# HITSZ-NRSL/De6D

Measured on AMD Instinct MI355X. Metric: scenes/sec (16384-pt KITTI) at 1/2/4/8 MI355X; 3D mAP parity vs ref, higher is better.
Workload: dtype f32

## Files before the change

### de6d_amd/csrc/fps_multi.h

```cpp
#pragma once
#include "fps_common.h"

namespace {

constexpr int kCandMax = 4;
constexpr int kWaves = 16, kSlots = 16;
constexpr int kMaxPicks = 32;
constexpr int kCoopMaxPicks = 64;
static_assert(kWaves * kCandMax == 64, "one sequencer lane per candidate");

template <int LO, int HI, int N>
__device__ __forceinline__ void sq_select(int ws, const float (&px)[N], const float (&py)[N], const float (&pz)[N],
                                          float &x, float &y, float &z) {
  if constexpr (HI - LO == 1) {
    x = px[LO]; y = py[LO]; z = pz[LO];
    asm volatile("" : "+v"(x), "+v"(y), "+v"(z));
  } else {
    constexpr int MID = (LO + HI) / 2;
    if (ws < MID) sq_select<LO, MID>(ws, px, py, pz, x, y, z);
    else sq_select<MID, HI>(ws, px, py, pz, x, y, z);
  }
}

template <int LO, int HI, int N>
__device__ __forceinline__ void sq_select5(int ws, const float (&px)[N], const float (&py)[N], const float (&pz)[N],
                                           const float (&pt)[N], const float (&pw)[N], float &x, float &y, float &z, float &t, float &w) {
  if constexpr (HI - LO == 1) {
    x = px[LO]; y = py[LO]; z = pz[LO]; t = pt[LO]; w = pw[LO];
    asm volatile("" : "+v"(x), "+v"(y), "+v"(z), "+v"(t), "+v"(w));
  } else {
    constexpr int MID = (LO + HI) / 2;
    if (ws < MID) sq_select5<LO, MID>(ws, px, py, pz, pt, pw, x, y, z, t, w);
    else sq_select5<MID, HI>(ws, px, py, pz, pt, pw, x, y, z, t, w);
  }
}

__device__ __forceinline__ void sq_quad_max2(float a, float b, float &ra, float &rb) {
  asm volatile(
      "s_nop 1\n\t"
      "v_max_f32_dpp %0, %2, %2 quad_perm:[1,0,3,2] row_mask:0xf bank_mask:0xf\n\t"
      "v_max_f32_dpp %1, %3, %3 quad_perm:[1,0,3,2] row_mask:0xf bank_mask:0xf\n\t"
      "s_nop 0\n\t"
      "v_max_f32_dpp %0, %0, %0 quad_perm:[2,3,0,1] row_mask:0xf bank_mask:0xf\n\t"
      "v_max_f32_dpp %1, %1, %1 quad_perm:[2,3,0,1] row_mask:0xf bank_mask:0xf\n\t"
      "s_nop 1\n\t"
      : "=&v"(ra), "=&v"(rb)
      : "v"(a), "v"(b));
}

__device__ __forceinline__ float sq_quad_max(float a) {
  float r;
  asm volatile(
      "s_nop 1\n\t"
      "v_max_f32_dpp %0, %1, %1 quad_perm:[1,0,3,2] row_mask:0xf bank_mask:0xf\n\t"
      "s_nop 1\n\t"
      "v_max_f32_dpp %0, %0, %0 quad_perm:[2,3,0,1] row_mask:0xf bank_mask:0xf\n\t"
      "s_nop 1\n\t"
      : "=&v"(r)
      : "v"(a));
  return r;
}

__device__ __forceinline__ float sq_pair_max(float a) {
  float r;
  asm volatile(
      "s_nop 1\n\t"
      "v_max_f32_dpp %0, %1, %1 quad_perm:[1,0,3,2] row_mask:0xf bank_mask:0xf\n\t"
      "s_nop 1\n\t"
      : "=&v"(r)
      : "v"(a));
  return r;
}
template <int K, int N>
__device__ __forceinline__ void sq_group_max_n(const float (&a)[N], float (&r)[N]) {
  static_assert(N == 1 || N == 2 || N == 4, "values per call");
  if constexpr (N == 4) {
    if constexpr (K == 2) {
      asm volatile("s_nop 1\n\t"
                   "v_max_f32_dpp %0, %4, %4 quad_perm:[1,0,3,2] row_mask:0xf bank_mask:0xf\n\t"
                   "v_max_f32_dpp %1, %5, %5 quad_perm:[1,0,3,2] row_mask:0xf bank_mask:0xf\n\t"
                   "v_max_f32_dpp %2, %6, %6 quad_perm:[1,0,3,2] row_mask:0xf bank_mask:0xf\n\t"
                   "v_max_f32_dpp %3, %7, %7 quad_perm:[1,0,3,2] row_mask:0xf bank_mask:0xf\n\t"
                   "s_nop 1\n\t"
                   : "=&v"(r[0]), "=&v"(r[1]), "=&v"(r[2]), "=&v"(r[3])
                   : "v"(a[0]), "v"(a[1]), "v"(a[2]), "v"(a[3]));
    } else {
      asm volatile("s_nop 1\n\t"
                   "v_max_f32_dpp %0, %4, %4 quad_perm:[1,0,3,2] row_mask:0xf bank_mask:0xf\n\t"
                   "v_max_f32_dpp %1, %5, %5 quad_perm:[1,0,3,2] row_mask:0xf bank_mask:0xf\n\t"
                   "v_max_f32_dpp %2, %6, %6 quad_perm:[1,0,3,2] row_mask:0xf bank_mask:0xf\n\t"
                   "v_max_f32_dpp %3, %7, %7 quad_perm:[1,0,3,2] row_mask:0xf bank_mask:0xf\n\t"
                   "v_max_f32_dpp %0, %0, %0 quad_perm:[2,3,0,1] row_mask:0xf bank_mask:0xf\n\t"
                   "v_max_f32_dpp %1, %1, %1 quad_perm:[2,3,0,1] row_mask:0xf bank_mask:0xf\n\t"
                   "v_max_f32_dpp %2, %2, %2 quad_perm:[2,3,0,1] row_mask:0xf bank_mask:0xf\n\t"
                   "v_max_f32_dpp %3, %3, %3 quad_perm:[2,3,0,1] row_mask:0xf bank_mask:0xf\n\t"
                   "s_nop 1\n\t"
                   : "=&v"(r[0]), "=&v"(r[1]), "=&v"(r[2]), "=&v"(r[3])
                   : "v"(a[0]), "v"(a[1]), "v"(a[2]), "v"(a[3]));
    }
  } else if constexpr (N == 2) {
    if constexpr (K == 2) {
      asm volatile("s_nop 1\n\t"
                   "v_max_f32_dpp %0, %2, %2 quad_perm:[1,0,3,2] row_mask:0xf bank_mask:0xf\n\t"
                   "v_max_f32_dpp %1, %3, %3 quad_perm:[1,0,3,2] row_mask:0xf bank_mask:0xf\n\t"
                   "s_nop 1\n\t"
                   : "=&v"(r[0]), "=&v"(r[1]) : "v"(a[0]), "v"(a[1]));
    } else {
      sq_quad_max2(a[0], a[1], r[0], r[1]);
    }
  } else {
    if constexpr (K == 2) r[0] = sq_pair_max(a[0]);
    else r[0] = sq_quad_max(a[0]);
  }
}

template <int K>
__device__ __forceinline__ float sq_group_max(float a) {
  if constexpr (K == 2) return sq_pair_max(a);
  else return sq_quad_max(a);
}

template <int K>
__device__ __forceinline__ unsigned sq_group_max_u32(unsigned a) {
  unsigned r;
  if constexpr (K == 2)
    asm volatile("s_nop 1\n\t"
                 "v_max_u32_dpp %0, %1, %1 quad_perm:[1,0,3,2] row_mask:0xf bank_mask:0xf\n\t"
                 "s_nop 1\n\t"
                 : "=&v"(r) : "v"(a));
  else
    asm volatile("s_nop 1\n\t"
                 "v_max_u32_dpp %0, %1, %1 quad_perm:[1,0,3,2] row_mask:0xf bank_mask:0xf\n\t"
                 "s_nop 1\n\t"
                 "v_max_u32_dpp %0, %0, %0 quad_perm:[2,3,0,1] row_mask:0xf bank_mask:0xf\n\t"
                 "s_nop 1\n\t"
                 : "=&v"(r) : "v"(a));
  return r;
}

__device__ __forceinline__ unsigned sq_wave_max_u32(unsigned v) {
  unsigned t;
  asm volatile(
      "s_nop 1\n\t"
      "v_max_u32_dpp %0, %1, %1 quad_perm:[1,0,3,2] row_mask:0xf bank_mask:0xf\n\t"
      "s_nop 1\n\t"
      "v_max_u32_dpp %0, %0, %0 quad_perm:[2,3,0,1] row_mask:0xf bank_mask:0xf\n\t"
      "s_nop 1\n\t"
      "v_max_u32_dpp %0, %0, %0 row_half_mirror row_mask:0xf bank_mask:0xf\n\t"
      "s_nop 1\n\t"
      "v_max_u32_dpp %0, %0, %0 row_mirror row_mask:0xf bank_mask:0xf\n\t"
      "s_nop 1\n\t"
      "v_max_u32_dpp %0, %0, %0 row_bcast:15 row_mask:0xa bank_mask:0xf\n\t"
      "s_nop 1\n\t"
      "v_max_u32_dpp %0, %0, %0 row_bcast:31 row_mask:0xc bank_mask:0xf\n\t"
      "s_nop 1\n\t"
      : "=&v"(t)
      : "v"(v));
  return (unsigned)__builtin_amdgcn_readlane((int)t, 63);
}

__device__ __forceinline__ void sq_wave_max2(float a, float b, float &ra, float &rb) {
  float ta, tb;
  asm volatile(
      "s_nop 1\n\t"
      "v_max_f32_dpp %0, %2, %2 quad_perm:[1,0,3,2] row_mask:0xf bank_mask:0xf\n\t"
      "v_max_f32_dpp %1, %3, %3 quad_perm:[1,0,3,2] row_mask:0xf bank_mask:0xf\n\t"
      "s_nop 0\n\t"
      "v_max_f32_dpp %0, %0, %0 quad_perm:[2,3,0,1] row_mask:0xf bank_mask:0xf\n\t"
      "v_max_f32_dpp %1, %1, %1 quad_perm:[2,3,0,1] row_mask:0xf bank_mask:0xf\n\t"
      "s_nop 0\n\t"
      "v_max_f32_dpp %0, %0, %0 row_half_mirror row_mask:0xf bank_mask:0xf\n\t"
      "v_max_f32_dpp %1, %1, %1 row_half_mirror row_mask:0xf bank_mask:0xf\n\t"
      "s_nop 0\n\t"
      "v_max_f32_dpp %0, %0, %0 row_mirror row_mask:0xf bank_mask:0xf\n\t"
      "v_max_f32_dpp %1, %1, %1 row_mirror row_mask:0xf bank_mask:0xf\n\t"
      "s_nop 0\n\t"
      "v_max_f32_dpp %0, %0, %0 row_bcast:15 row_mask:0xa bank_mask:0xf\n\t"
      "v_max_f32_dpp %1, %1, %1 row_bcast:15 row_mask:0xa bank_mask:0xf\n\t"
      "s_nop 0\n\t"
      "v_max_f32_dpp %0, %0, %0 row_bcast:31 row_mask:0xc bank_mask:0xf\n\t"
      "v_max_f32_dpp %1, %1, %1 row_bcast:31 row_mask:0xc bank_mask:0xf\n\t"
      "s_nop 1\n\t"
      : "=&v"(ta), "=&v"(tb)
      : "v"(a), "v"(b));
  ra = d6_readlane_f(ta, 63);
  rb = d6_readlane_f(tb, 63);
}

struct SqRecords {
  float v[64], x[64], y[64], z[64];
  int k[64];
  int nc[kWaves];
};

struct SqRecordsW {
  float t[64], w[64];
};

template <int SG>
__device__ __forceinline__ void sq_hide_lane_duplicates(const float (&px)[SG], const float (&py)[SG], const float (&pz)[SG],
                                                        float (&pt)[SG]) {
#pragma unroll
  for (int j = 1; j < SG; ++j) {
    bool dup = false;
#pragma unroll
    for (int i = 0; i < j; ++i) dup |= px[i] == px[j] && py[i] == py[j] && pz[i] == pz[j];
    pt[j] = dup ? 0.f : pt[j];
  }
}

template <int SG>
__device__ __forceinline__ void sq_hide_lane_duplicates_w(const float (&px)[SG], const float (&py)[SG], const float (&pz)[SG],
                                                          const float (&pw)[SG], float (&pt)[SG]) {
#pragma unroll
  for (int j = 1; j < SG; ++j) {
    bool dup = false;
#pragma unroll
    for (int i = 0; i < j; ++i) dup |= px[i] == px[j] && py[i] == py[j] && pz[i] == pz[j] && pw[i] == pw[j];
    pt[j] = dup ? 0.f : pt[j];
  }
}

template <int SG>
__device__ __forceinline__ void sq_apply(float cx, float cy, float cz, const float (&px)[SG], const float (&py)[SG],
                                         const float (&pz)[SG], float (&pt)[SG]) {
  const fps_f32x2 c2x = {cx, cx}, c2y = {cy, cy}, c2z = {cz, cz};
#pragma unroll
  for (int q = 0; q < SG / 2; ++q) {
    const int s0 = 2 * q;
    const fps_f32x2 dx = fps_f32x2{px[s0], px[s0 + 1]} - c2x;
    const fps_f32x2 dy = fps_f32x2{py[s0], py[s0 + 1]} - c2y;
    const fps_f32x2 dz = fps_f32x2{pz[s0], pz[s0 + 1]} - c2z;
    fps_f32x2 d = dy * dy;
    d = __builtin_elementwise_fma(dx, dx, d);
    d = __builtin_elementwise_fma(dz, dz, d);
    pt[s0] = d6_vmin(d[0], pt[s0]);
    pt[s0 + 1] = d6_vmin(d[1], pt[s0 + 1]);
  }
}

template <int SG, int kCand>
__device__ __forceinline__ float sq_rescan(float cx, float cy, float cz, int log2s, const float (&px)[SG], const float (&py)[SG],
                                           const float (&pz)[SG], float (&pt)[SG], const unsigned short *korig_w, SqRecords &rec,
                                           int wave, int depth = kCand) {
  const int lane = threadIdx.x & 63;
  float best = -1.0f, sec = -1.0f;
  int bs = 0;
  const fps_f32x2 c2x = {cx, cx}, c2y = {cy, cy}, c2z = {cz, cz};
  auto visit = [&](int j, float d) {
    const float t = d6_vmin(d, pt[j]);
    pt[j] = t;
    sec = __builtin_amdgcn_fmed3f(best, sec, t);
    const bool up = t > best;
    bs = up ? j : bs;
    best = d6_vmax(best, t);
  };
#pragma unroll
  for (int q = 0; q < SG / 2; ++q) {
    const int s0 = 2 * q;
    const fps_f32x2 dx = fps_f32x2{px[s0], px[s0 + 1]} - c2x;
    const fps_f32x2 dy = fps_f32x2{py[s0], py[s0 + 1]} - c2y;
    const fps_f32x2 dz = fps_f32x2{pz[s0], pz[s0 + 1]} - c2z;
    fps_f32x2 d = dy * dy;
    d = __builtin_elementwise_fma(dx, dx, d);
    d = __builtin_elementwise_fma(dz, dz, d);
    visit(s0, d[0]);
    visit(s0 + 1, d[1]);
  }
  static_assert(SG % 2 == 0, "slot pairs");
  auto second_slot = [&]() -> int {
    float target = sec;
    int skip = bs;
    asm volatile("" : "+v"(target), "+v"(skip));
    int ss = 0;
#pragma unroll
    for (int j = SG - 1; j >= 0; --j) ss = (pt[j] == target && j != skip) ? j : ss;
    return ss;
  };

  int taken = 0;
  float head = best;
  float cmax = 0.f;
  int nc = 0;
#pragma nounroll
  for (int i = 0; i < depth; ++i) {
    const float wm = d6_wave_max(head);
    if (i == 0) cmax = wm;
    const u64 tie = __ballot(head == wm);
    int wl = __builtin_ctzll(tie);
    int ss = 0;
    bool have_ss = false;
    if (__popcll(tie) != 1) {
      if (__ballot(taken != 0 && head == wm) != 0ull) { ss = second_slot(); have_ss = true; }
      const int hs = taken ? ss : bs;
      wl = fps_min_key_lane(tie, fps_tie_key((int)korig_w[lane * SG + hs], log2s));
    }
    const int wtk = d6_readlane_i(taken, wl);
    int ws;
    if (wtk == 0) {
      ws = d6_readlane_i(bs, wl);
    } else {
      if (!have_ss) ss = second_slot();
      ws = d6_readlane_i(ss, wl);
    }
    if (lane == wl) {
      float x, y, z;
      sq_select<0, SG>(ws, px, py, pz, x, y, z);
      const int o = wave * kCandMax + i;
      rec.v[o] = wm;
      rec.k[o] = (int)korig_w[lane * SG + ws];
      rec.x[o] = x; rec.y[o] = y; rec.z[o] = z;
      taken = 1;
      head = sec;
    }
    nc = i + 1;
    if (wtk != 0) break;
  }
  if (lane == 0) rec.nc[wave] = nc;
  return cmax;
}

template <int SG, int kCand>
__device__ __forceinline__ float sq_rescan_w(float cx, float cy, float cz, int log2s, const float (&px)[SG], const float (&py)[SG],
                                             const float (&pz)[SG], const float (&pw)[SG], float (&pt)[SG],
                                             const unsigned short *korig_w, SqRecords &rec, SqRecordsW &recw, int wave,
                                             int depth = kCand) {
  const int lane = threadIdx.x & 63;
  float best = -1.0f, sec = -1.0f, tm = 0.f;
  int bs = 0;
  const fps_f32x2 c2x = {cx, cx}, c2y = {cy, cy}, c2z = {cz, cz};
  auto visit = [&](int j, float d) {
    const float t = d6_vmin(d, pt[j]);
    pt[j] = t;
    tm = d6_vmax(tm, t);
    const float sc = t * pw[j];
    sec = __builtin_amdgcn_fmed3f(best, sec, sc);
    const bool up = sc > best;
    bs = up ? j : bs;
    best = d6_vmax(best, sc);
  };
#pragma unroll
  for (int q = 0; q < SG / 2; ++q) {
    const int s0 = 2 * q;
    const fps_f32x2 dx = fps_f32x2{px[s0], px[s0 + 1]} - c2x;
    const fps_f32x2 dy = fps_f32x2{py[s0], py[s0 + 1]} - c2y;
    const fps_f32x2 dz = fps_f32x2{pz[s0], pz[s0 + 1]} - c2z;
    fps_f32x2 d = dy * dy;
    d = __builtin_elementwise_fma(dx, dx, d);
    d = __builtin_elementwise_fma(dz, dz, d);
    visit(s0, d[0]);
    visit(s0 + 1, d[1]);
  }
  auto second_slot = [&]() -> int {
    float target = sec;
    int skip = bs;
    asm volatile("" : "+v"(target), "+v"(skip));
    int ss = 0;
#pragma unroll
    for (int j = SG - 1; j >= 0; --j) ss = (pt[j] * pw[j] == target && j != skip) ? j : ss;
    return ss;
  };
  int taken = 0;
  float head = best;
  int nc = 0;
#pragma nounroll
  for (int i = 0; i < depth; ++i) {
    const float wm = d6_wave_max(head);
    const u64 tie = __ballot(head == wm);
    int wl = __builtin_ctzll(tie);
    int ss = 0;
    bool have_ss = false;
    if (__popcll(tie) != 1) {
      if (__ballot(taken != 0 && head == wm) != 0ull) { ss = second_slot(); have_ss = true; }
      const int hs = taken ? ss : bs;
      wl = fps_min_key_lane(tie, fps_tie_key((int)korig_w[lane * SG + hs], log2s));
    }
    const int wtk = d6_readlane_i(taken, wl);
    int ws;
    if (wtk == 0) {
      ws = d6_readlane_i(bs, wl);
    } else {
      if (!have_ss) ss = second_slot();
      ws = d6_readlane_i(ss, wl);
    }
    if (lane == wl) {
      float x, y, z, t, w;
      sq_select5<0, SG>(ws, px, py, pz, pt, pw, x, y, z, t, w);
      const int o = wave * kCandMax + i;
      rec.v[o] = wm;
      rec.k[o] = (int)korig_w[lane * SG + ws];
      rec.x[o] = x; rec.y[o] = y; rec.z[o] = z;
      recw.t[o] = t; recw.w[o] = w;
      taken = 1;
      head = sec;
    }
    nc = i + 1;
    if (wtk != 0) break;
  }
  if (lane == 0) rec.nc[wave] = nc;
  return d6_wave_max(tm);
}

}
```

### de6d_amd/csrc/fps_seq.hip

```cpp
#include <stdio.h>
#include "fps_common.h"
#include "fps_multi.h"

namespace {

#ifdef DET6D_EXPERIMENTS
__device__ unsigned long long d6_fps_seq_stats[16];
#define SQ_STAT(i, v) do { const unsigned long long sv_ = (unsigned long long)(v); if (blockIdx.x == 0 && (threadIdx.x & 63) == 0) atomicAdd(&sq_stats_lds[i], sv_); } while (0)
#else
#define SQ_STAT(i, v) do { } while (0)
#endif

template <int kCand, int SG = kSlots>
__global__ __launch_bounds__(1024) void fps_seq_kernel(int n, int m, int log2s, long long xyz_bstride, long long idx_bstride,
                                                       int idx_add, const float *__restrict__ xyz,
                                                       const int *__restrict__ perm, int *__restrict__ idxs, int max_picks, int depth_add) {
  __shared__ unsigned short korig[64 * kWaves * SG];
  __shared__ SqRecords rec;
  __shared__ float pick_x[kMaxPicks], pick_y[kMaxPicks], pick_z[kMaxPicks];
  __shared__ int pick_n;
#ifdef DET6D_EXPERIMENTS
  __shared__ unsigned long long sq_stats_lds[16];
  if (threadIdx.x < 16) sq_stats_lds[threadIdx.x] = 0ull;
  const long long t_begin = clock64();
#endif
  const int h = threadIdx.x, lane = h & 63;
  const int wave = __builtin_amdgcn_readfirstlane(h >> 6);
  xyz += (size_t)blockIdx.x * xyz_bstride;
  perm += (size_t)blockIdx.x * n;
  idxs += (size_t)blockIdx.x * idx_bstride;
  unsigned short *korig_w = korig + (size_t)wave * 64 * SG;

  float px[SG], py[SG], pz[SG], pt[SG];
  float lox, loy, loz, hix, hiy, hiz;
  {
    float ax = 3.0e38f, ay = 3.0e38f, az = 3.0e38f, bx = -3.0e38f, by = -3.0e38f, bz = -3.0e38f;
#pragma unroll
    for (int j = 0; j < SG; ++j) {
      const int pos = (wave * 64 + lane) * SG + j;
      const int k = perm[pos];
      korig[pos] = (unsigned short)k;
      px[j] = xyz[(size_t)k * 3 + 0];
      py[j] = xyz[(size_t)k * 3 + 1];
      pz[j] = xyz[(size_t)k * 3 + 2];
      asm volatile("" : "+v"(px[j]), "+v"(py[j]), "+v"(pz[j]));
      pt[j] = 1e10f;
      ax = d6_vmin(ax, px[j]); bx = d6_vmax(bx, px[j]);
      ay = d6_vmin(ay, py[j]); by = d6_vmax(by, py[j]);
      az = d6_vmin(az, pz[j]); bz = d6_vmax(bz, pz[j]);
    }
    lox = d6_wave_min(ax); hix = d6_wave_max(bx);
    loy = d6_wave_min(ay); hiy = d6_wave_max(by);
    loz = d6_wave_min(az); hiz = d6_wave_max(bz);
  }
  sq_hide_lane_duplicates<SG>(px, py, pz, pt);
  float cmax = __builtin_inff();
  if (h == 0) { pick_x[0] = xyz[0]; pick_y[0] = xyz[1]; pick_z[0] = xyz[2]; pick_n = 1; idxs[0] = idx_add; }
  __syncthreads();

  int r = 1;
  while (true) {
#ifdef DET6D_EXPERIMENTS
    const long long ta0 = clock64();
#endif
    {
      const int np = pick_n;
      const float sx = pick_x[lane & (kMaxPicks - 1)], sy = pick_y[lane & (kMaxPicks - 1)], sz = pick_z[lane & (kMaxPicks - 1)];
      const float gx = fmaxf(0.f, fmaxf(lox - sx, sx - hix));
      const float gy = fmaxf(0.f, fmaxf(loy - sy, sy - hiy));
      const float gz = fmaxf(0.f, fmaxf(loz - sz, sz - hiz));
      const float lb = d6_sqdist(gx, gy, gz);
      u64 need = __ballot(lane < np && (r == 1 || !(lb >= cmax)));
      if (need != 0ull) {
        while (need & (need - 1ull)) {
          const int i = __builtin_ctzll(need);
          need &= need - 1ull;
          sq_apply<SG>(d6_readlane_f(sx, i), d6_readlane_f(sy, i), d6_readlane_f(sz, i), px, py, pz, pt);
          SQ_STAT(3, 1);
        }
        const int i = __builtin_ctzll(need);
        SQ_STAT(2, 1);
        cmax = sq_rescan<SG, kCand>(d6_readlane_f(sx, i), d6_readlane_f(sy, i), d6_readlane_f(sz, i), log2s, px, py, pz, pt, korig_w, rec, wave,
                                    np <= depth_add ? min(kCand, 2) : kCand);
      }
    }
    if (r >= m) break;
#ifdef DET6D_EXPERIMENTS
    const long long ta1 = clock64();
    if (wave == 0) SQ_STAT(6, ta1 - ta0);
    if (wave == 5) SQ_STAT(7, ta1 - ta0);
#endif
    __syncthreads();
#ifdef DET6D_EXPERIMENTS
    const long long tb0 = clock64();
    if (wave == 0) SQ_STAT(8, tb0 - ta1);
#endif
    if (wave == 0) {
      SQ_STAT(0, 1);
      constexpr int LOG2K = kCand == 2 ? 1 : 2;
      const bool live = lane < kWaves * kCand;
      const int region = live ? lane >> LOG2K : 0;
      const int nc = rec.nc[region];
      const int slot = lane & (kCand - 1);
      const int o = region * kCandMax + slot;
      float cv = live && slot < nc ? rec.v[o] : -1.0f;
      const float qx = rec.x[o], qy = rec.y[o], qz = rec.z[o];
      const int kidx = rec.k[o];
      const bool is_last = live && slot == nc - 1;
      const float bound_v = sq_group_max<kCand>(is_last ? cv : -2.0f);
      const unsigned ub = ((__builtin_bit_cast(unsigned, bound_v) << 1) | 1u) + 2u;
      const bool alive = live && slot < nc;
      const unsigned ntk = ~fps_tie_key(kidx, log2s);
      const unsigned ntk_last = sq_group_max_u32<kCand>(is_last ? ntk : 0u);
      const unsigned thr = !alive ? 0xFFFFFFFFu : ntk >= ntk_last ? ub - 1u : ub;
      const unsigned alt = is_last ? ub : 0u;
      int j = 0;
      const int jmax = min(max_picks, m - r);
      int mwl = 0;
      {
        bool go;
        do {
          const unsigned ekey = (__builtin_bit_cast(unsigned, cv) << 1) + 2u;
          const unsigned key = ekey >= thr ? ekey : alt;
          const unsigned best = sq_wave_max_u32(key);
          const u64 tie = __ballot(key == best);
          int wl = __builtin_ctzll(tie);
          if (__popcll(tie) != 1) wl = fps_min_key_lane(tie, ~ntk);
          const float sx = d6_readlane_f(qx, wl), sy = d6_readlane_f(qy, wl), sz = d6_readlane_f(qz, wl);
          mwl = lane == j ? wl : mwl;
          cv = d6_vmin(cv, d6_sqdist(qx - sx, qy - sy, qz - sz));
          go = (best & 1u) == 0u;
          j += go ? 1 : 0;
#ifdef DET6D_EXPERIMENTS
          if (!go) SQ_STAT(4, 1);
#endif
        } while (go && j < jmax);
      }
      {
        const float mx = __shfl(qx, mwl), my = __shfl(qy, mwl), mz = __shfl(qz, mwl);
        const int mk = __shfl(kidx, mwl);
        if (lane < j) {
          pick_x[lane] = mx; pick_y[lane] = my; pick_z[lane] = mz;
          idxs[r + lane] = mk + idx_add;
        }
      }
      if (lane == 0) pick_n = j;
      SQ_STAT(1, j);
#ifdef DET6D_EXPERIMENTS
      SQ_STAT(9, clock64() - tb0);
#endif
    }
    __syncthreads();
    r += pick_n;
  }
#ifdef DET6D_EXPERIMENTS
  if (wave == 0) {
    SQ_STAT(5, clock64() - t_begin);
    __builtin_amdgcn_s_waitcnt(0);
    if (blockIdx.x == 0 && lane < 16) d6_fps_seq_stats[lane] = sq_stats_lds[lane];
  }
#endif
}

template <int kCand, int SG>
__global__ __launch_bounds__(1024) void fps_seq_w_kernel(int n, int m, int log2s, long long xyz_bstride, long long idx_bstride,
                                                         int idx_add, const float *__restrict__ xyz, const int *__restrict__ perm,
                                                         int *__restrict__ idxs, int max_picks, int depth_add,
                                                         const float *__restrict__ weights, long long w_bstride, float gamma,
                                                         int w_is_score, int *__restrict__ flags) {
  __shared__ unsigned short korig[64 * kWaves * SG];
  __shared__ SqRecords rec;
  __shared__ SqRecordsW recw;
  __shared__ float pick_x[kMaxPicks], pick_y[kMaxPicks], pick_z[kMaxPicks];
  __shared__ int pick_n;
  __shared__ float w0_val[kWaves], w0_x[kWaves], w0_y[kWaves], w0_z[kWaves];
  __shared__ unsigned w0_key[kWaves];
  __shared__ int small_any;
  const int h = threadIdx.x, lane = h & 63;
  const int wave = __builtin_amdgcn_readfirstlane(h >> 6);
  xyz += (size_t)blockIdx.x * xyz_bstride;
  perm += (size_t)blockIdx.x * n;
  idxs += (size_t)blockIdx.x * idx_bstride;
  weights += (size_t)blockIdx.x * w_bstride;
  flags += (size_t)blockIdx.x * n;
  unsigned short *korig_w = korig + (size_t)wave * 64 * SG;
  if (h == 0) small_any = 0;

  float px[SG], py[SG], pz[SG], pt[SG], pw[SG];
  float lox, loy, loz, hix, hiy, hiz;
  bool small = false;
  {
    float ax = 3.0e38f, ay = 3.0e38f, az = 3.0e38f, bx = -3.0e38f, by = -3.0e38f, bz = -3.0e38f;
#pragma unroll
    for (int j = 0; j < SG; ++j) {
      const int pos = (wave * 64 + lane) * SG + j;
      const int k = perm[pos];
      korig[pos] = (unsigned short)k;
      px[j] = xyz[(size_t)k * 3 + 0];
      py[j] = xyz[(size_t)k * 3 + 1];
      pz[j] = xyz[(size_t)k * 3 + 2];
      float w = weights[k];
      if (w_is_score) w = d6_sigmoid_powf(w, gamma);
      pw[j] = w;
      small = small || !((double)w >= 1e-12);
      asm volatile("" : "+v"(px[j]), "+v"(py[j]), "+v"(pz[j]), "+v"(pw[j]));
      pt[j] = 1e10f;
      ax = d6_vmin(ax, px[j]); bx = d6_vmax(bx, px[j]);
      ay = d6_vmin(ay, py[j]); by = d6_vmax(by, py[j]);
      az = d6_vmin(az, pz[j]); bz = d6_vmax(bz, pz[j]);
    }
    lox = d6_wave_min(ax); hix = d6_wave_max(bx);
    loy = d6_wave_min(ay); hiy = d6_wave_max(by);
    loz = d6_wave_min(az); hiz = d6_wave_max(bz);
  }
  __syncthreads();
  if (__ballot(small) != 0ull && lane == 0) small_any = 1;
  {
    float bw = pw[0];
    int bs0 = 0;
#pragma unroll
    for (int j = 1; j < SG; ++j) {
      const bool up = pw[j] > bw;
      bs0 = up ? j : bs0;
      bw = up ? pw[j] : bw;
    }
    const float wm = d6_wave_max(small ? 0.f : bw);
    const u64 tie = __ballot(bw == wm);
    int wl = tie ? __builtin_ctzll(tie) : 0;
    const unsigned mykey = fps_tie_key((int)korig_w[lane * SG + bs0], log2s);
    if (__popcll(tie) > 1) wl = fps_min_key_lane(tie, mykey);
    if (lane == wl) {
      float x, y, z;
      sq_select<0, SG>(bs0, px, py, pz, x, y, z);
      w0_val[wave] = bw; w0_key[wave] = mykey; w0_x[wave] = x; w0_y[wave] = y; w0_z[wave] = z;
    }
  }
  __syncthreads();
  if (h == 0) flags[0] = small_any;
  if (small_any) return;
  if (wave == 0) {
    const bool mine = lane < kWaves;
    const float v = mine ? w0_val[lane & (kWaves - 1)] : -1.0f;
    const unsigned key = mine ? w0_key[lane & (kWaves - 1)] : 0xFFFFFFFFu;
    const float vm = d6_wave_max(v);
    const u64 tie = __ballot(mine && v == vm);
    int wl = __builtin_ctzll(tie);
    if (__popcll(tie) > 1) wl = fps_min_key_lane(tie, key);
    if (lane == wl) {
      pick_x[0] = w0_x[lane]; pick_y[0] = w0_y[lane]; pick_z[0] = w0_z[lane];
      pick_n = 1;
      idxs[0] = fps_tie_key_point(key, log2s) + idx_add;
    }
  }
  sq_hide_lane_duplicates_w<SG>(px, py, pz, pw, pt);
  float cmax = __builtin_inff();
  __syncthreads();

  int r = 1;
  while (true) {
    {
      const int np = pick_n;
      const float sx = pick_x[lane & (kMaxPicks - 1)], sy = pick_y[lane & (kMaxPicks - 1)], sz = pick_z[lane & (kMaxPicks - 1)];
      const float gx = fmaxf(0.f, fmaxf(lox - sx, sx - hix));
      const float gy = fmaxf(0.f, fmaxf(loy - sy, sy - hiy));
      const float gz = fmaxf(0.f, fmaxf(loz - sz, sz - hiz));
      const float lb = d6_sqdist(gx, gy, gz);
      u64 need = __ballot(lane < np && (r == 1 || !(lb >= cmax)));
      if (need != 0ull) {
        while (need & (need - 1ull)) {
          const int i = __builtin_ctzll(need);
          need &= need - 1ull;
          sq_apply<SG>(d6_readlane_f(sx, i), d6_readlane_f(sy, i), d6_readlane_f(sz, i), px, py, pz, pt);
        }
        const int i = __builtin_ctzll(need);
        cmax = sq_rescan_w<SG, kCand>(d6_readlane_f(sx, i), d6_readlane_f(sy, i), d6_readlane_f(sz, i), log2s, px, py, pz, pw, pt, korig_w,
                                      rec, recw, wave, np <= depth_add ? min(kCand, 2) : kCand);
      }
    }
    if (r >= m) break;
    __syncthreads();
    if (wave == 0) {
      constexpr int LOG2K = kCand == 2 ? 1 : 2;
      const bool live = lane < kWaves * kCand;
      const int region = live ? lane >> LOG2K : 0;
      const int nc = rec.nc[region];
      const int slot = lane & (kCand - 1);
      const int o = region * kCandMax + slot;
      const bool alive = live && slot < nc;
      float cv = alive ? recw.t[o] : -1.0f;
      const float cw = alive ? recw.w[o] : 1.0f;
      const float sv = alive ? rec.v[o] : -1.0f;
      const float qx = rec.x[o], qy = rec.y[o], qz = rec.z[o];
      const int kidx = rec.k[o];
      const bool is_last = live && slot == nc - 1;
      const float bound_v = sq_group_max<kCand>(is_last ? sv : -2.0f);
      const unsigned ub = ((__builtin_bit_cast(unsigned, bound_v) << 1) | 1u) + 2u;
      const unsigned ntk = ~fps_tie_key(kidx, log2s);
      const unsigned ntk_last = sq_group_max_u32<kCand>(is_last ? ntk : 0u);
      const unsigned thr = !alive ? 0xFFFFFFFFu : ntk >= ntk_last ? ub - 1u : ub;
      const unsigned alt = is_last ? ub : 0u;
      int j = 0;
      const int jmax = min(max_picks, m - r);
      int mwl = 0;
      {
        bool go;
        do {
          const unsigned ekey = (__builtin_bit_cast(unsigned, cv * cw) << 1) + 2u;
          const unsigned key = ekey >= thr ? ekey : alt;
          const unsigned best = sq_wave_max_u32(key);
          const u64 tie = __ballot(key == best);
          int wl = __builtin_ctzll(tie);
          if (__popcll(tie) != 1) wl = fps_min_key_lane(tie, ~ntk);
          const float sx = d6_readlane_f(qx, wl), sy = d6_readlane_f(qy, wl), sz = d6_readlane_f(qz, wl);
          mwl = lane == j ? wl : mwl;
          cv = d6_vmin(cv, d6_sqdist(qx - sx, qy - sy, qz - sz));
          go = (best & 1u) == 0u;
          j += go ? 1 : 0;
        } while (go && j < jmax);
      }
      {
        const float mx = __shfl(qx, mwl), my = __shfl(qy, mwl), mz = __shfl(qz, mwl);
        const int mk = __shfl(kidx, mwl);
        if (lane < j) {
          pick_x[lane] = mx; pick_y[lane] = my; pick_z[lane] = mz;
          idxs[r + lane] = mk + idx_add;
        }
      }
      if (lane == 0) pick_n = j;
    }
    __syncthreads();
    r += pick_n;
  }
}

}

#ifdef DET6D_EXPERIMENTS
extern "C" __attribute__((visibility("default"))) int det6d_dbg_fps_seq_stats(unsigned long long *out_host) {
  return hipMemcpyFromSymbol(out_host, HIP_SYMBOL(d6_fps_seq_stats), sizeof(unsigned long long) * 16) == hipSuccess ? 0 : -1;
}

namespace {
__device__ unsigned d6_poison_sink;
__global__ __launch_bounds__(1024) void poison_lds_kernel(unsigned pattern, unsigned words) {
  extern __shared__ unsigned lds[];
  for (unsigned i = threadIdx.x; i < words; i += 1024) lds[i] = pattern;
  __syncthreads();
  if (lds[(threadIdx.x * 97u) % words] != pattern) d6_poison_sink = 1u;
}
}
void det6d_dbg_poison_lds_hook(hipStream_t stream) {
  static const char *env = getenv("DET6D_DBG_POISON_LDS");
  if (!env) return;
  static const unsigned pattern = (unsigned)strtoul(env, nullptr, 0);
  const unsigned bytes = 160u * 1024u;
  DET6D_MAX_DYNAMIC_LDS(poison_lds_kernel, bytes);
  hipLaunchKernelGGL(poison_lds_kernel, dim3(1024), dim3(1024), bytes, stream, pattern, bytes / 4u);
  const hipError_t rc = hipGetLastError();
  if (rc != hipSuccess) fprintf(stderr, "det6d_dbg_poison_lds_hook: %s\n", hipGetErrorString(rc));
}
namespace {
__global__ __launch_bounds__(1024) void probe_lds_kernel(unsigned *out) {
  __shared__ unsigned probe[8192];
  unsigned v = probe[threadIdx.x * 8];
  asm volatile("" : "+v"(v));
  out[blockIdx.x * 1024 + threadIdx.x] = v;
}
}
extern "C" __attribute__((visibility("default"))) int det6d_dbg_probe_lds(unsigned *out, int blocks, void *stream) {
  det6d_dbg_poison_lds_hook((hipStream_t)stream);
  hipLaunchKernelGGL(probe_lds_kernel, dim3(blocks), dim3(1024), 0, (hipStream_t)stream, out);
  return det6d_check_launch("det6d_dbg_probe_lds");
}
#endif

#ifdef DET6D_EXPERIMENTS
namespace {
template <int R>
__global__ __launch_bounds__(1024) void occupy_kernel(int usec, float *sink) {
  extern __shared__ float occ_lds[];
  float r[R];
#pragma unroll
  for (int i = 0; i < R; ++i) r[i] = (float)(threadIdx.x + i);
  const unsigned long long t0 = wall_clock64();
  while (wall_clock64() - t0 < (unsigned long long)usec * 100ull) {
    __builtin_amdgcn_s_sleep(100);
#pragma unroll
    for (int i = 0; i < R; ++i) asm volatile("" : "+v"(r[i]));
  }
  float s = 0.f;
#pragma unroll
  for (int i = 0; i < R; ++i) s += r[i];
  if (s == -1.f) { occ_lds[threadIdx.x] = s; sink[0] = occ_lds[0]; }
}
}
extern "C" __attribute__((visibility("default"))) int det6d_dbg_occupy(int blocks, int regs, int lds, int usec, float *sink, void *stream) {
  hipStream_t s = (hipStream_t)stream;
#define D6_OCC(R)                                                         \
  do {                                                                    \
    DET6D_MAX_DYNAMIC_LDS(occupy_kernel<R>, 160 * 1024);                  \
    hipLaunchKernelGGL(occupy_kernel<R>, dim3(blocks), dim3(1024), lds, s, usec, sink); \
  } while (0)
  if (regs >= 96) D6_OCC(96); else if (regs >= 80) D6_OCC(80); else if (regs >= 56) D6_OCC(56); else if (regs >= 40) D6_OCC(40); else D6_OCC(16);
#undef D6_OCC
  return det6d_check_launch("det6d_dbg_occupy");
}
#endif

int det6d_fps_seq_launch(int b, int n, int m, int log2s, long long xyz_bstride, long long idx_bstride, int idx_add,
                         const float *xyz, const int *perm, int *idx, hipStream_t stream) {
  if (n != 16384 && n != 4096) return DET6D_EINVAL;
  static const int max_picks_env = det6d_env_int("DET6D_FPS_SEQ_PICKS", kMaxPicks);
  static const int cands = det6d_env_int("DET6D_FPS_SEQ_CANDS", 4);
  static const int depth_add = det6d_env_int("DET6D_FPS_SEQ_DEPTH_ADD", 1);
  const int max_picks = max_picks_env < 1 ? 1 : max_picks_env > kMaxPicks ? kMaxPicks : max_picks_env;
#ifdef DET6D_EXPERIMENTS
  det6d_dbg_poison_lds_hook(stream);
#endif
  if (n == 4096)
    hipLaunchKernelGGL((fps_seq_kernel<4, 4>), dim3(b), dim3(1024), 0, stream, n, m, log2s, xyz_bstride, idx_bstride, idx_add, xyz, perm, idx, max_picks, depth_add);
  else if (cands == 2)
    hipLaunchKernelGGL((fps_seq_kernel<2>), dim3(b), dim3(1024), 0, stream, n, m, log2s, xyz_bstride, idx_bstride, idx_add, xyz, perm, idx, max_picks, depth_add);
  else
    hipLaunchKernelGGL((fps_seq_kernel<4>), dim3(b), dim3(1024), 0, stream, n, m, log2s, xyz_bstride, idx_bstride, idx_add, xyz, perm, idx, max_picks, depth_add);
  return det6d_check_launch("det6d_fps (multi-pick)");
}

int det6d_fps_seq_w_launch(int b, int n, int m, int log2s, long long xyz_bstride, long long idx_bstride, int idx_add,
                           const float *xyz, const int *perm, int *idx, const float *weights, long long w_bstride, float gamma,
                           int w_is_score, int *flags, hipStream_t stream) {
  if (n != 16384 && n != 4096) return DET6D_EINVAL;
  static const int max_picks_env = det6d_env_int("DET6D_FPS_SEQ_PICKS", kMaxPicks);
  static const int depth_add = det6d_env_int("DET6D_FPS_SEQ_DEPTH_ADD", 1);
  const int max_picks = max_picks_env < 1 ? 1 : max_picks_env > kMaxPicks ? kMaxPicks : max_picks_env;
#ifdef DET6D_EXPERIMENTS
  det6d_dbg_poison_lds_hook(stream);
#endif
  if (n == 4096)
    hipLaunchKernelGGL((fps_seq_w_kernel<4, 4>), dim3(b), dim3(1024), 0, stream, n, m, log2s, xyz_bstride, idx_bstride, idx_add, xyz, perm,
                       idx, max_picks, depth_add, weights, w_bstride, gamma, w_is_score, flags);
  else
    hipLaunchKernelGGL((fps_seq_w_kernel<4, 16>), dim3(b), dim3(1024), 0, stream, n, m, log2s, xyz_bstride, idx_bstride, idx_add, xyz, perm,
                       idx, max_picks, depth_add, weights, w_bstride, gamma, w_is_score, flags);
  return det6d_check_launch("det6d_fps (multi-pick, score-weighted)");
}
```

Baseline: 12780.

## Move FPS per-slot min-distances to LDS with double-buffered register staging

```diff
diff --git a/de6d_amd/csrc/fps_multi.h b/de6d_amd/csrc/fps_multi.h
--- a/de6d_amd/csrc/fps_multi.h
+++ b/de6d_amd/csrc/fps_multi.h
@@ -197,6 +197,51 @@
   float t[64], w[64];
 };
 
+constexpr int kLdsDistStride = 1024;
+constexpr int kLdsDistChunk = 4;
+struct SqLdsDist {
+  float *p;
+  float st[2 * kLdsDistChunk];
+};
+__device__ __forceinline__ constexpr int sq_stage(int j) { return ((j / kLdsDistChunk) & 1) * kLdsDistChunk + j % kLdsDistChunk; }
+
+template <int N>
+__device__ __forceinline__ float sq_dist_get(const float (&t)[N], int j) { return t[j]; }
+template <int N>
+__device__ __forceinline__ void sq_dist_set(float (&t)[N], int j, float v) { t[j] = v; }
+__device__ __forceinline__ float sq_dist_get(const SqLdsDist &t, int j) { return t.p[j * kLdsDistStride]; }
+__device__ __forceinline__ void sq_dist_set(SqLdsDist &t, int j, float v) { t.p[j * kLdsDistStride] = v; }
+
+template <int N>
+__device__ __forceinline__ void sq_sweep_open(float (&)[N]) {}
+template <int N>
+__device__ __forceinline__ float sq_sweep_get(const float (&t)[N], int j) { return t[j]; }
+template <int N>
+__device__ __forceinline__ void sq_sweep_set(float (&t)[N], int j, float v) { t[j] = v; }
+__device__ __forceinline__ void sq_sweep_open(SqLdsDist &t) {
+#pragma unroll
+  for (int j = 0; j < 2 * kLdsDistChunk; ++j) t.st[sq_stage(j)] = sq_dist_get(t, j);
+  asm volatile("" ::: "memory");
+}
+__device__ __forceinline__ float sq_sweep_get(const SqLdsDist &t, int j) { return t.st[sq_stage(j)]; }
+__device__ __forceinline__ void sq_sweep_set(SqLdsDist &t, int j, float v) { t.st[sq_stage(j)] = v; }
+template <int SG>
+__device__ __forceinline__ void sq_sweep_next(SqLdsDist &t, int j) {
+  static_assert(SG % kLdsDistChunk == 0 && SG >= 2 * kLdsDistChunk, "whole chunks, two in flight");
+  if ((j + 1) % kLdsDistChunk != 0) return;
+  const int c0 = j + 1 - kLdsDistChunk;
+  asm volatile("" ::: "memory");
+#pragma unroll
+  for (int i = 0; i < kLdsDistChunk; ++i) sq_dist_set(t, c0 + i, t.st[sq_stage(c0 + i)]);
+  if (c0 + 2 * kLdsDistChunk < SG) {
+#pragma unroll
+    for (int i = 0; i < kLdsDistChunk; ++i) t.st[sq_stage(c0 + i)] = sq_dist_get(t, c0 + 2 * kLdsDistChunk + i);
+  }
+  asm volatile("" ::: "memory");
+}
+template <int SG, int N>
+__device__ __forceinline__ void sq_sweep_next(float (&)[N], int) {}
+
 template <int SG>
 __device__ __forceinline__ void sq_hide_lane_duplicates(const float (&px)[SG], const float (&py)[SG], const float (&pz)[SG],
                                                         float (&pt)[SG]) {
@@ -208,6 +253,18 @@
     pt[j] = dup ? 0.f : pt[j];
   }
 }
+template <int SG, class PT>
+__device__ __forceinline__ void sq_init_hiding_lane_duplicates(const float (&px)[SG], const float (&py)[SG],
+                                                               const float (&pz)[SG], PT &pt, float fresh) {
+  sq_dist_set(pt, 0, fresh);
+#pragma unroll
+  for (int j = 1; j < SG; ++j) {
+    bool dup = false;
+#pragma unroll
+    for (int i = 0; i < j; ++i) dup |= px[i] == px[j] && py[i] == py[j] && pz[i] == pz[j];
+    sq_dist_set(pt, j, dup ? 0.f : fresh);
+  }
+}
 
 template <int SG>
 __device__ __forceinline__ void sq_hide_lane_duplicates_w(const float (&px)[SG], const float (&py)[SG], const float (&pz)[SG],
@@ -221,10 +278,11 @@
   }
 }
 
-template <int SG>
+template <int SG, class PT>
 __device__ __forceinline__ void sq_apply(float cx, float cy, float cz, const float (&px)[SG], const float (&py)[SG],
-                                         const float (&pz)[SG], float (&pt)[SG]) {
+                                         const float (&pz)[SG], PT &pt) {
   const fps_f32x2 c2x = {cx, cx}, c2y = {cy, cy}, c2z = {cz, cz};
+  sq_sweep_open(pt);
 #pragma unroll
   for (int q = 0; q < SG / 2; ++q) {
     const int s0 = 2 * q;
@@ -234,27 +292,29 @@
     fps_f32x2 d = dy * dy;
     d = __builtin_elementwise_fma(dx, dx, d);
     d = __builtin_elementwise_fma(dz, dz, d);
-    pt[s0] = d6_vmin(d[0], pt[s0]);
-    pt[s0 + 1] = d6_vmin(d[1], pt[s0 + 1]);
-  }
-}
-
-template <int SG, int kCand>
+    sq_sweep_set(pt, s0, d6_vmin(d[0], sq_sweep_get(pt, s0)));
+    sq_sweep_set(pt, s0 + 1, d6_vmin(d[1], sq_sweep_get(pt, s0 + 1)));
+    sq_sweep_next<SG>(pt, s0 + 1);
+  }
+}
+
+template <int SG, int kCand, class PT>
 __device__ __forceinline__ float sq_rescan(float cx, float cy, float cz, int log2s, const float (&px)[SG], const float (&py)[SG],
-                                           const float (&pz)[SG], float (&pt)[SG], const unsigned short *korig_w, SqRecords &rec,
+                                           const float (&pz)[SG], PT &pt, const unsigned short *korig_w, SqRecords &rec,
                                            int wave, int depth = kCand) {
   const int lane = threadIdx.x & 63;
   float best = -1.0f, sec = -1.0f;
   int bs = 0;
   const fps_f32x2 c2x = {cx, cx}, c2y = {cy, cy}, c2z = {cz, cz};
   auto visit = [&](int j, float d) {
-    const float t = d6_vmin(d, pt[j]);
-    pt[j] = t;
+    const float t = d6_vmin(d, sq_sweep_get(pt, j));
+    sq_sweep_set(pt, j, t);
     sec = __builtin_amdgcn_fmed3f(best, sec, t);
     const bool up = t > best;
     bs = up ? j : bs;
     best = d6_vmax(best, t);
   };
+  sq_sweep_open(pt);
 #pragma unroll
   for (int q = 0; q < SG / 2; ++q) {
     const int s0 = 2 * q;
@@ -266,6 +326,7 @@
     d = __builtin_elementwise_fma(dz, dz, d);
     visit(s0, d[0]);
     visit(s0 + 1, d[1]);
+    sq_sweep_next<SG>(pt, s0 + 1);
   }
   static_assert(SG % 2 == 0, "slot pairs");
   auto second_slot = [&]() -> int {
@@ -274,7 +335,7 @@
     asm volatile("" : "+v"(target), "+v"(skip));
     int ss = 0;
 #pragma unroll
-    for (int j = SG - 1; j >= 0; --j) ss = (pt[j] == target && j != skip) ? j : ss;
+    for (int j = SG - 1; j >= 0; --j) ss = (sq_dist_get(pt, j) == target && j != skip) ? j : ss;
     return ss;
   };
 
diff --git a/de6d_amd/csrc/fps_seq.hip b/de6d_amd/csrc/fps_seq.hip
--- a/de6d_amd/csrc/fps_seq.hip
+++ b/de6d_amd/csrc/fps_seq.hip
@@ -1,4 +1,5 @@
 #include <stdio.h>
+#include <type_traits>
 #include "fps_common.h"
 #include "fps_multi.h"
 
@@ -11,10 +12,10 @@
 #define SQ_STAT(i, v) do { } while (0)
 #endif
 
-template <int kCand, int SG = kSlots>
-__global__ __launch_bounds__(1024) void fps_seq_kernel(int n, int m, int log2s, long long xyz_bstride, long long idx_bstride,
-                                                       int idx_add, const float *__restrict__ xyz,
-                                                       const int *__restrict__ perm, int *__restrict__ idxs, int max_picks, int depth_add) {
+template <int kCand, int SG>
+__device__ __forceinline__ void fps_seq_body(int n, int m, int log2s, long long xyz_bstride, long long idx_bstride,
+                                             int idx_add, const float *__restrict__ xyz,
+                                             const int *__restrict__ perm, int *__restrict__ idxs, int max_picks, int depth_add) {
   __shared__ unsigned short korig[64 * kWaves * SG];
   __shared__ SqRecords rec;
   __shared__ float pick_x[kMaxPicks], pick_y[kMaxPicks], pick_z[kMaxPicks];
@@ -31,7 +32,14 @@
   idxs += (size_t)blockIdx.x * idx_bstride;
   unsigned short *korig_w = korig + (size_t)wave * 64 * SG;
 
-  float px[SG], py[SG], pz[SG], pt[SG];
+  float px[SG], py[SG], pz[SG];
+  constexpr bool kDistInLds = SG == kSlots;
+  typename std::conditional<kDistInLds, SqLdsDist, float[SG]>::type pt;
+  if constexpr (kDistInLds) {
+    __shared__ float dist[SG * kLdsDistStride];
+    static_assert(kLdsDistStride == 64 * kWaves, "one word per thread and slot");
+    pt.p = dist + h;
+  }
   float lox, loy, loz, hix, hiy, hiz;
   {
     float ax = 3.0e38f, ay = 3.0e38f, az = 3.0e38f, bx = -3.0e38f, by = -3.0e38f, bz = -3.0e38f;
@@ -44,7 +52,7 @@
       py[j] = xyz[(size_t)k * 3 + 1];
       pz[j] = xyz[(size_t)k * 3 + 2];
       asm volatile("" : "+v"(px[j]), "+v"(py[j]), "+v"(pz[j]));
-      pt[j] = 1e10f;
+      if constexpr (!kDistInLds) pt[j] = 1e10f;
       ax = d6_vmin(ax, px[j]); bx = d6_vmax(bx, px[j]);
       ay = d6_vmin(ay, py[j]); by = d6_vmax(by, py[j]);
       az = d6_vmin(az, pz[j]); bz = d6_vmax(bz, pz[j]);
@@ -53,7 +61,8 @@
     loy = d6_wave_min(ay); hiy = d6_wave_max(by);
     loz = d6_wave_min(az); hiz = d6_wave_max(bz);
   }
-  sq_hide_lane_duplicates<SG>(px, py, pz, pt);
+  if constexpr (kDistInLds) sq_init_hiding_lane_duplicates<SG>(px, py, pz, pt, 1e10f);
+  else sq_hide_lane_duplicates<SG>(px, py, pz, pt);
   float cmax = __builtin_inff();
   if (h == 0) { pick_x[0] = xyz[0]; pick_y[0] = xyz[1]; pick_z[0] = xyz[2]; pick_n = 1; idxs[0] = idx_add; }
   __syncthreads();
@@ -162,12 +171,27 @@
 #endif
 }
 
+template <int kCand, int SG = kSlots>
+__global__ __launch_bounds__(1024) __attribute__((amdgpu_num_vgpr(44))) void fps_seq_kernel(
+    int n, int m, int log2s, long long xyz_bstride, long long idx_bstride, int idx_add, const float *__restrict__ xyz,
+    const int *__restrict__ perm, int *__restrict__ idxs, int max_picks, int depth_add) {
+  static_assert(SG == kSlots, "the 4-slot kernel is the specialisation below");
+  fps_seq_body<kCand, SG>(n, m, log2s, xyz_bstride, idx_bstride, idx_add, xyz, perm, idxs, max_picks, depth_add);
+}
+template <>
+__global__ __launch_bounds__(1024) __attribute__((amdgpu_num_vgpr(64))) void fps_seq_kernel<4, 4>(int n, int m, int log2s, long long xyz_bstride, long long idx_bstride,
+                                                             int idx_add, const float *__restrict__ xyz,
+                                                             const int *__restrict__ perm, int *__restrict__ idxs, int max_picks,
+                                                             int depth_add) {
+  fps_seq_body<4, 4>(n, m, log2s, xyz_bstride, idx_bstride, idx_add, xyz, perm, idxs, max_picks, depth_add);
+}
+
 template <int kCand, int SG>
 __global__ __launch_bounds__(1024) void fps_seq_w_kernel(int n, int m, int log2s, long long xyz_bstride, long long idx_bstride,
-                                                         int idx_add, const float *__restrict__ xyz, const int *__restrict__ perm,
+                                                         int idx_add, const float *__restrict__ xyz, const int *perm,
                                                          int *__restrict__ idxs, int max_picks, int depth_add,
                                                          const float *__restrict__ weights, long long w_bstride, float gamma,
-                                                         int w_is_score, int *__restrict__ flags) {
+                                                         int w_is_score, int *flags) {
   __shared__ unsigned short korig[64 * kWaves * SG];
   __shared__ SqRecords rec;
   __shared__ SqRecordsW recw;
```

Result: no change. 12730, median of 2 (-0.4%).
